# google-research/simclr

Measured on AMD Instinct MI355X. Metric: images/sec (whole node), ResNet-50 1x SimCLR pretraining step @224px, higher is better.
Workload: dtype f32; 1 GPU; ResNet-50 1x, 224x224, 2 views/image, per-GPU batch 512, global batch 512, NT-Xent T=0.1 + linear-eval head + LARS, global BN, dp1; global_batch=512, parallelism=dp1

## Files before the change

### simclr_amd/csrc/conv.hip

```cpp
#include "common.h"
#include <stdlib.h>
#include <string.h>
#include <mutex>
#include <type_traits>

namespace {

enum { MODE_FWD = 0, MODE_DGRAD = 1 };

struct ConvP {
  const void* x;
  const void* w;
  void* y;
  float* stats;
  int V, IH, IW, IC, OH, OW, N, KH, KW, stride, pad;
  int pixpitch;
  int M, K;
  int nslot, accumulate;
  int m_tiles, n_tiles;
  int cs, py, px, cls_h, cls_w;
  int ntaps;
  int taps[9];
  unsigned long long tap_w, dy_w, dx_w;
  const void* bn_x;
  const void* bn_mask;
  const float *bn_scale, *bn_shift, *bn_mean, *bn_rstd;
  int bn_mode;
  const void* x2;
  const float* bias;
  int ic2, pixpitch2;
  int win_j, win_bytes;
  int fapply;
  const void* zero;
  int diag;
  int split;
  const float* pivot;
  int rem_full, rem_tiles, rem_parts;
  float* part_ws;
  unsigned* part_flags;
  unsigned* part_err;
  int w_ps;
  int x_ps;
  unsigned x_bytes;
  int rs_dq[3], rs_drow[3], rs_dcol[3];
};

#ifdef SIMCLR_DIAG
#define DIAG(b) ((p.diag & (b)) != 0)
#else
#define DIAG(b) false
#endif

template <typename T> struct MMA;
template <> struct MMA<uint16_t> {
  __device__ static __forceinline__ f32x4 run(const u32x4& a, const u32x4& b, f32x4 c) {
    return __builtin_amdgcn_mfma_f32_16x16x32_bf16(__builtin_bit_cast(bf16x8, a),
                                                   __builtin_bit_cast(bf16x8, b), c, 0, 0, 0);
  }
};
template <> struct MMA<float> {
  __device__ static __forceinline__ f32x4 run(const u32x4& a, const u32x4& b, f32x4 c) {
#pragma unroll
    for (int j = 0; j < 4; ++j)
      c = __builtin_amdgcn_mfma_f32_16x16x4f32(__uint_as_float(a[j]), __uint_as_float(b[j]), c, 0, 0, 0);
    return c;
  }
};

__device__ __forceinline__ void split_terms2(const u32x4& c0, const u32x4& c1, u32x4& hi, u32x4& lo) {
#pragma unroll
  for (int j = 0; j < 4; ++j) {
    const float x0 = __uint_as_float(j < 2 ? c0[2 * j] : c1[2 * j - 4]), x1 = __uint_as_float(j < 2 ? c0[2 * j + 1] : c1[2 * j - 3]);
    const uint32_t h = pack_bf16x2(x0, x1);
    hi[j] = h;
    lo[j] = pack_bf16x2(x0 - __uint_as_float(h << 16), x1 - __uint_as_float(h & 0xffff0000u));
  }
}
__device__ __forceinline__ void split_terms3(const u32x4& c0, const u32x4& c1, u32x4& hi, u32x4& lo, u32x4& lo2) {
#pragma unroll
  for (int j = 0; j < 4; ++j) {
    const float x0 = __uint_as_float(j < 2 ? c0[2 * j] : c1[2 * j - 4]), x1 = __uint_as_float(j < 2 ? c0[2 * j + 1] : c1[2 * j - 3]);
    const uint32_t h = pack_bf16x2(x0, x1);
    const float r0 = x0 - __uint_as_float(h << 16), r1 = x1 - __uint_as_float(h & 0xffff0000u);
    const uint32_t l = pack_bf16x2(r0, r1);
    hi[j] = h;
    lo[j] = l;
    lo2[j] = pack_bf16x2(r0 - __uint_as_float(l << 16), r1 - __uint_as_float(l & 0xffff0000u));
  }
}
__device__ __forceinline__ f32x4 mma_bf16(const u32x4& a, const u32x4& b, f32x4 c) {
  return __builtin_amdgcn_mfma_f32_16x16x32_bf16(__builtin_bit_cast(bf16x8, a), __builtin_bit_cast(bf16x8, b), c, 0, 0, 0);
}
typedef __attribute__((ext_vector_type(8))) _Float16 f16x8;
#define F16_WSCALE_LOG2 8
__device__ __forceinline__ void split_terms2_f16(const u32x4& c0, const u32x4& c1, u32x4& hi, u32x4& lo) {
#pragma unroll
  for (int j = 0; j < 4; ++j) {
    const float x0 = __uint_as_float(j < 2 ? c0[2 * j] : c1[2 * j - 4]), x1 = __uint_as_float(j < 2 ? c0[2 * j + 1] : c1[2 * j - 3]);
    uint32_t h, l;
    split_pair<true>(x0, x1, h, l);
    hi[j] = h; lo[j] = l;
  }
}
__device__ __forceinline__ f32x4 mma_f16(const u32x4& a, const u32x4& b, f32x4 c) {
  return __builtin_amdgcn_mfma_f32_16x16x32_f16(__builtin_bit_cast(f16x8, a), __builtin_bit_cast(f16x8, b), c, 0, 0, 0);
}
template <int NA, int NB, bool TR, int terms, bool PSA = false, bool PSB2 = false, typename LA, typename LB>
__device__ __forceinline__ void mma_f32_chunks(f32x4* __restrict__ accp, LA lda, LB ldb) {
  static_assert(terms == 0 || terms == 3 || terms == 6 || terms == 13, "0 = exact fp32, 3 / 6 = split-bf16 terms, 13 = three split-fp16 terms");
  static_assert(!(PSA || PSB2) || terms == 3 || terms == 13, "pre-split operand: two planes (hi, lo) = the three-term products only");
#define acc_(i, j) accp[TR ? (j) * NA + (i) : (i) * NB + (j)]
  if constexpr (terms == 0) {
#pragma unroll
    for (int ks = 0; ks < 2; ++ks) {
      u32x4 a[NA], b[NB];
#pragma unroll
      for (int i = 0; i < NA; ++i) a[i] = lda(i, ks);
#pragma unroll
      for (int j = 0; j < NB; ++j) b[j] = ldb(j, ks);
#pragma unroll
      for (int i = 0; i < NA; ++i)
#pragma unroll
        for (int j = 0; j < NB; ++j)
#pragma unroll
          for (int e = 0; e < 4; ++e)
            acc_(i, j) = __builtin_amdgcn_mfma_f32_16x16x4f32(__uint_as_float(a[i][e]), __uint_as_float(b[j][e]), acc_(i, j), 0, 0, 0);
    }
// ... 1149 lines not shown
                const u32x2 mv = *(const u32x2*)((const uint16_t*)p.bn_mask + off + n);
                mk[0] = __uint_as_float(mv[0] << 16); mk[1] = __uint_as_float(mv[0] & 0xffff0000u);
                mk[2] = __uint_as_float(mv[1] << 16); mk[3] = __uint_as_float(mv[1] & 0xffff0000u);
              }
            } else {
              const float4 sc = *(const float4*)(bnp + nl), sh = *(const float4*)(bnp + BN + nl);
              mk[0] = fmaf(xf[0], sc.x, sh.x); mk[1] = fmaf(xf[1], sc.y, sh.y);
              mk[2] = fmaf(xf[2], sc.z, sh.z); mk[3] = fmaf(xf[3], sc.w, sh.w);
            }
            const float4 mu = *(const float4*)(bnp + 2 * BN + nl), rs = *(const float4*)(bnp + 3 * BN + nl);
            const float mua[4] = {mu.x, mu.y, mu.z, mu.w}, rsa[4] = {rs.x, rs.y, rs.z, rs.w};
#pragma unroll
            for (int r = 0; r < 4; ++r) {
              v[r] = mk[r] > 0.f ? v[r] : 0.f;
              st_s[ni][r] += v[r];
              st_q[ni][r] += v[r] * (xf[r] - mua[r]) * rsa[r];
            }
          }
          if (sizeof(T) == 4) {
            *(float4*)dst = make_float4(v[0], v[1], v[2], v[3]);
          } else {
            u32x2 pk; pk[0] = pack_bf16x2(v[0], v[1]); pk[1] = pack_bf16x2(v[2], v[3]);
            *(u32x2*)dst = pk;
          }
        }
      }
    }
    }
  }
  if (ROWSTATS) {
    __syncthreads();
    float* red = WSUM ? (float*)wred : (float*)smem;
    constexpr int NRED = WSUM ? NW : RPP;
    if (!WSUM) {
#pragma unroll
      for (int e = 0; e < 8; ++e) {
        red[((tid / CPR) * BN + e_cc * 8 + e) * 2] = e_s[e];
        red[((tid / CPR) * BN + e_cc * 8 + e) * 2 + 1] = e_q[e];
      }
      __syncthreads();
    }
    const bool own_slot = p.nslot >= mslots;
    if (tid < BN && n0 + tid < p.N && (count > 0 || own_slot)) {
      float s1 = 0.f, s2 = 0.f;
      for (int w = 0; w < NRED; ++w) { s1 += red[(w * BN + tid) * 2]; s2 += red[(w * BN + tid) * 2 + 1]; }
      if (BNEPI) s2 = (s2 - bnp[2 * BN + tid] * s1) * bnp[3 * BN + tid];
      float* st = p.stats + (long long)(own_slot ? mslot : mslot % p.nslot) * 2 * p.N;
      if (own_slot) { st[n0 + tid] = s1; st[p.N + n0 + tid] = s2; }
      else { atomicAdd(st + n0 + tid, s1); atomicAdd(st + p.N + n0 + tid, s2); }
    }
    return;
  }
  if (STATS) {
    __syncthreads();
    float* red = (float*)smem;
#pragma unroll
    for (int ni = 0; ni < NI; ++ni) {
#pragma unroll
      for (int r = 0; r < 4; ++r) {
        float s = st_s[ni][r], ss = st_q[ni][r];
#pragma unroll
        for (int o = 1; o < 16; o <<= 1) { s += __shfl_xor(s, o, 64); ss += __shfl_xor(ss, o, 64); }
        if (fl == 0) {
          const int nl = wn * 64 + ni * 16 + g * 4 + r;
          red[(wm * BN + nl) * 2] = s;
          red[(wm * BN + nl) * 2 + 1] = ss;
        }
      }
    }
    __syncthreads();
    const bool own_slot = p.nslot >= mslots;
    if (tid < BN && n0 + tid < p.N && (count > 0 || own_slot)) {
      float s = 0.f, ss = 0.f;
#pragma unroll
      for (int w = 0; w < WM; ++w) { s += red[(w * BN + tid) * 2]; ss += red[(w * BN + tid) * 2 + 1]; }
      float* st = p.stats + (long long)(own_slot ? mslot : mslot % p.nslot) * 2 * p.N;
      if (own_slot) { st[n0 + tid] = s; st[p.N + n0 + tid] = ss; }
      else { atomicAdd(st + n0 + tid, s); atomicAdd(st + p.N + n0 + tid, ss); }
    }
  }
}

#include "igemm_wide.h"

struct WgradP {
  const void* x;
  const void* dy;
  float* dw;
  int V, IH, IW, IC, OH, OW, N, KH, KW, stride, pad, pixpitch;
  int M, K, splits, chunks_per_split;
  int k_tiles, n_tiles;
  int xcd_map;
  const void* zero;
  int diag;
  int split;
  int dy_ps;
};

typedef __attribute__((ext_vector_type(4))) short s16x4_t;
typedef __attribute__((address_space(3))) s16x4_t lds_s16x4_t;

template <typename T> __device__ __forceinline__ int px_key(int px) {
  return sizeof(T) == 2 ? ((px & 3) | (((px >> 3) & 1) << 2)) : (((px & 3) << 1) | ((px >> 2) & 1));
}

template <typename T, int BKW, int BNW, bool MT = false>
__global__ __launch_bounds__(256) void conv_wgrad(const WgradP p) {
  constexpr int EPC = Elem<T>::EPC;
  constexpr int BR = 8 * EPC;
  constexpr int WK = 2;
  constexpr int WNN = 2;
  constexpr int KI = BKW / WK / 16;
  constexpr int NI = BNW / WNN / 16;
  constexpr int A_CPR = BKW / EPC;
  constexpr int B_CPR = BNW / EPC;
  constexpr int A_CH = BR * A_CPR / 256;
  constexpr int B_CH = BR * B_CPR / 256;
  constexpr int A_RB = BKW * sizeof(T);
  constexpr int B_RB = BNW * sizeof(T);
  constexpr int A_BLK = A_RB / 32;
  constexpr int B_BLK = B_RB / 32;
  constexpr int BUF = BR * (A_RB + B_RB);
  extern __shared__ __attribute__((aligned(16))) unsigned char smem[];

  const int tid = threadIdx.x, lane = tid & 63;
  const int wave = __builtin_amdgcn_readfirstlane(tid >> 6);
  const int g = lane >> 4, fl = lane & 15;
  const int wk = wave / WNN, wn = wave % WNN;
  const int tiles = p.k_tiles * p.n_tiles;
  int tile, split;
  if (p.xcd_map) {
    const int xcd = blockIdx.x & 7, bidx = blockIdx.x >> 3;
    tile = bidx % tiles;
    split = (bidx / tiles) * 8 + xcd;
  } else {
    tile = blockIdx.x % tiles;
    split = blockIdx.x / tiles;
  }
  if (split >= p.splits) return;
  const int ktile = tile % p.k_tiles;
  const int ntile = tile / p.k_tiles;
  const int kk0 = ktile * BKW;
  const int tap = kk0 / p.IC, ci0 = kk0 - tap * p.IC;
  const int ty = tap / p.KW, tx = tap - ty * p.KW;
  const int n0 = ntile * BNW;
  const T* __restrict__ X = (const T*)p.x;
  const T* __restrict__ DY = (const T*)p.dy;

  f32x4 acc[KI][NI];
#pragma unroll
  for (int i = 0; i < KI; ++i)
#pragma unroll
    for (int j = 0; j < NI; ++j) acc[i][j] = (f32x4){0.f, 0.f, 0.f, 0.f};

  const int nchunks = (p.M + BR - 1) / BR;
  const int c_begin = split * p.chunks_per_split;
  const int c_end = min(nchunks, c_begin + p.chunks_per_split);

  u32x4 ra[A_CH], rb[B_CH];
#ifdef SIMCLR_DIAG
#pragma unroll
  for (int j = 0; j < A_CH; ++j) ra[j] = zero16();
#pragma unroll
  for (int j = 0; j < B_CH; ++j) rb[j] = zero16();
#endif
  const bool flat = p.KH == 1 && p.KW == 1 && p.stride == 1 && p.pad == 0 && p.IH == p.OH && p.IW == p.OW;
// ... 1439 lines not shown
__global__ __launch_bounds__(256) void presplit_packed(const float4* __restrict__ src, u32x4* __restrict__ dst, long long npix) {
  for (long long i = blockIdx.x * 256ll + threadIdx.x; i < npix; i += (long long)gridDim.x * 256ll) {
    const float4 v = src[i];
    uint32_t h0, l0, h1, l1;
    split_pair<false>(v.x, v.y, h0, l0);
    split_pair<false>(v.z, v.w, h1, l1);
    dst[i] = (u32x4){h0, h1, l0, l1};
  }
}

__global__ void unpack_stem_dw(const float* __restrict__ src, float* __restrict__ dst, int KH, int KW,
                               int CI, int CO, int KWP, int accumulate) {
  const int total = KH * KW * CI * CO;
  for (int i = blockIdx.x * blockDim.x + threadIdx.x; i < total; i += gridDim.x * blockDim.x) {
    const int co = i % CO;
    const int ci = (i / CO) % CI;
    const int kw = (i / (CO * CI)) % KW;
    const int kh = i / (CO * CI * KW);
    const float v = src[(long long)((kh * KWP + kw) * 4 + ci) * CO + co];
    dst[i] = accumulate ? dst[i] + v : v;
  }
}

static int g_f32_terms_fwd = 0, g_f32_terms_bwd = 0;
static bool valid_terms(int t, bool fwd) { return t == 0 || t == 3 || t == 6 || (fwd && t == 13); }
static int terms_of(int* dtype, bool fwd) {
  const int f = (*dtype >> 12) & 0xff;
  *dtype &= ~(0xff << 12);
  if (f == 0) return fwd ? g_f32_terms_fwd : g_f32_terms_bwd;
  return valid_terms(f - 1, fwd) ? f - 1 : -1;
}

static bool take_ps_w(int* dtype) {
  const bool f = (*dtype & SIMCLR_FMT_PS_W) != 0;
  *dtype &= ~SIMCLR_FMT_PS_W;
  return f;
}

static thread_local char g_last_inst[512] = "";
static bool dry_run() { return simclr_dry_run(); }
template <typename T, int MODE> static void record_inst(const char* kern, unsigned grid, unsigned block, size_t lds, const ConvP& p) {
  snprintf(g_last_inst, sizeof(g_last_inst), "(%s) elt=%d role=%s grid=%u block=%u lds=%zu m_tiles=%d n_tiles=%d tail_parts=%d", kern,
           (int)sizeof(T), MODE == MODE_FWD ? "fwd" : "dgrad", grid, block, lds, p.m_tiles, p.n_tiles, p.rem_parts);
}
template <typename T> static const char* type_name() { return sizeof(T) == 2 ? "uint16_t" : "float"; }
static const char* mode_name(int mode) { return mode == MODE_FWD ? "MODE_FWD" : "MODE_DGRAD"; }
static const char* tf(bool v) { return v ? "true" : "false"; }

template <typename T, int MODE, int BN, bool STATS, bool GLDS>
static void run_igemm(dim3 grid, dim3 block, size_t lds, hipStream_t stream, const ConvP& p) {
  char name[128];
  snprintf(name, sizeof(name), "conv_igemm<%s, %s, %d, %s, %s>", type_name<T>(), mode_name(MODE), BN, tf(STATS), tf(GLDS));
  record_inst<T, MODE>(name, grid.x, block.x, lds, p);
  if (!dry_run()) hipLaunchKernelGGL((conv_igemm<T, MODE, BN, STATS, GLDS>), grid, block, lds, stream, p);
}

template <int MODE, bool STATS, bool BNEPI, bool FLAT>
static void run_wide(dim3 grid, dim3 block, size_t lds, hipStream_t stream, const ConvP& p) {
  char name[128];
  snprintf(name, sizeof(name), "conv_igemm_wide<%s, %s, %s, %s>", mode_name(MODE), tf(STATS), tf(BNEPI), tf(FLAT));
  record_inst<uint16_t, MODE>(name, grid.x, block.x, lds, p);
  if (!dry_run()) hipLaunchKernelGGL((conv_igemm_wide<MODE, STATS, BNEPI, FLAT>), grid, block, lds, stream, p);
}

template <typename T, int MODE, int BM, int BN, int NW, int STAGES, bool STATS, bool BNEPI, bool EXT = false,
          bool WIN = false, bool FAPPLY = false, int SPL = 0, bool TAIL = false, bool PSB = false, int FAS = 0, int EPS = 0, bool PSX = false>
static void run_persistent(dim3 grid, dim3 block, size_t lds, hipStream_t stream, const ConvP& p) {
  const int opt[9] = {EXT, WIN, FAPPLY, SPL, TAIL, PSB, FAS, EPS, PSX};
  const bool is_bool[9] = {true, true, true, false, true, true, false, false, true};
  int n = 9;
  while (n > 0 && opt[n - 1] == 0) --n;
  char name[256];
  int len = snprintf(name, sizeof(name), "conv_igemm_persistent<%s, %s, %d, %d, %d, %d, %s, %s", type_name<T>(), mode_name(MODE), BM, BN, NW,
                     STAGES, tf(STATS), tf(BNEPI));
  for (int i = 0; i < n; ++i)
    len += is_bool[i] ? snprintf(name + len, sizeof(name) - len, ", %s", tf(opt[i])) : snprintf(name + len, sizeof(name) - len, ", %d", opt[i]);
  snprintf(name + len, sizeof(name) - len, ">");
  record_inst<T, MODE>(name, grid.x, block.x, lds, p);
  if (!dry_run())
    hipLaunchKernelGGL((conv_igemm_persistent<T, MODE, BM, BN, NW, STAGES, STATS, BNEPI, EXT, WIN, FAPPLY, SPL, TAIL, PSB, FAS, EPS, PSX>),
                       grid, block, lds, stream, p);
}

struct WgradRec { int k_tiles, n_tiles, splits, chunks_per_split, xcd_map; };
static WgradRec rec_of(const WgradP& p) { return {p.k_tiles, p.n_tiles, p.splits, p.chunks_per_split, p.xcd_map}; }
static WgradRec rec_of(const Wgrad3P& p) { return {p.ci_tiles, p.co_tiles, p.splits, p.chunks_per_split, 1}; }
static WgradRec rec_of(const StemWgP& p) { return {1, 1, p.splits, p.chunks_per_split, 0}; }
static void record_wgrad(const char* kern, int elt, const char* role, unsigned grid, unsigned block, size_t lds, const WgradRec& r) {
  snprintf(g_last_inst, sizeof(g_last_inst), "(%s) elt=%d role=%s grid=%u block=%u lds=%zu k_tiles=%d n_tiles=%d splits=%d chunks_per_split=%d xcd_map=%d",
           kern, elt, role, grid, block, lds, r.k_tiles, r.n_tiles, r.splits, r.chunks_per_split, r.xcd_map);
}

template <typename T, int BKW, int BNW, bool MT = false>
static void run_wgrad(const char* role, unsigned grid, unsigned block, size_t lds, hipStream_t stream, const WgradP& p) {
  char name[128];
  snprintf(name, sizeof(name), MT ? "conv_wgrad<%s, %d, %d, true>" : "conv_wgrad<%s, %d, %d>", type_name<T>(), BKW, BNW);
  record_wgrad(name, (int)sizeof(T), role, grid, block, lds, rec_of(p));
  if (!dry_run()) hipLaunchKernelGGL((conv_wgrad<T, BKW, BNW, MT>), dim3(grid), dim3(block), lds, stream, p);
}

template <typename T, int BKW, int BNW, int BRM, int STAGES, int WK = 2, int WNN = 2, bool GRAM = false, bool MT = false, int SPL = 0, int PSD = 0>
static void run_wgrad_dma(const char* role, unsigned grid, unsigned block, size_t lds, hipStream_t stream, const WgradP& p) {
  const int opt[6] = {WK, WNN, GRAM, MT, SPL, PSD}, dflt[6] = {2, 2, 0, 0, 0, 0};
  const bool is_bool[6] = {false, false, true, true, false, false};
  int n = 6;
  while (n > 0 && opt[n - 1] == dflt[n - 1]) --n;
  char name[160];
  int len = snprintf(name, sizeof(name), "conv_wgrad_dma<%s, %d, %d, %d, %d", type_name<T>(), BKW, BNW, BRM, STAGES);
  for (int i = 0; i < n; ++i)
    len += is_bool[i] ? snprintf(name + len, sizeof(name) - len, ", %s", tf(opt[i])) : snprintf(name + len, sizeof(name) - len, ", %d", opt[i]);
  snprintf(name + len, sizeof(name) - len, ">");
  record_wgrad(name, (int)sizeof(T), role, grid, block, lds, rec_of(p));
  if (!dry_run())
    hipLaunchKernelGGL((conv_wgrad_dma<T, BKW, BNW, BRM, STAGES, WK, WNN, GRAM, MT, SPL, PSD>), dim3(grid), dim3(block), lds, stream, p);
}

template <int ST> static void run_wgrad3x3_bf16(unsigned grid, unsigned block, size_t lds, hipStream_t stream, const Wgrad3P& q) {
  char name[64];
  snprintf(name, sizeof(name), "conv_wgrad3x3_bf16<%d>", ST);
  record_wgrad(name, 2, "wgrad", grid, block, lds, rec_of(q));
  if (!dry_run()) hipLaunchKernelGGL(conv_wgrad3x3_bf16<ST>, dim3(grid), dim3(block), lds, stream, q);
}
static void run_wgrad3x3_f32ps(unsigned grid, unsigned block, size_t lds, hipStream_t stream, const Wgrad3P& q) {
  record_wgrad("conv_wgrad3x3_f32ps", 4, "wgrad", grid, block, lds, rec_of(q));
  if (!dry_run()) hipLaunchKernelGGL(conv_wgrad3x3_f32ps, dim3(grid), dim3(block), lds, stream, q);
}
template <int STAGES> static void run_stem_wgrad_ps(unsigned grid, unsigned block, size_t lds, hipStream_t stream, const StemWgP& p) {
  char name[64];
  snprintf(name, sizeof(name), "stem_wgrad_ps<7, 2, %d>", STAGES);
  record_wgrad(name, 4, "stem_wgrad_ps", grid, block, lds, rec_of(p));
  if (!dry_run()) hipLaunchKernelGGL((stem_wgrad_ps<7, 2, STAGES>), dim3(grid), dim3(block), lds, stream, p);
}
static void run_slab_reduce(const void* slabs, int splits, long long numel, float* out, int accumulate, hipStream_t stream) {
  const int grid = max(1, (int)ceil_div(numel / 4, 16));
  const size_t len = strlen(g_last_inst);
  snprintf(g_last_inst + len, sizeof(g_last_inst) - len, " reduce_grid=%d", grid);
  if (!dry_run()) hipLaunchKernelGGL(slab_reduce, dim3(grid), dim3(256), 0, stream, (const float*)slabs, splits, numel, out, accumulate);
}

static const void* zero_page() {
  static void* zp = nullptr;
  if (dry_run()) return (const void*)&g_last_inst;
  if (!zp && hipGetSymbolAddress(&zp, HIP_SYMBOL(g_zero16)) != hipSuccess) zp = nullptr;
  return zp;
}

static void igemm_persistent_grid(long long M, int N, int* bn, int* n_tiles, int* grid, bool narrow = false) {
  const int BN = (N <= 64 || narrow) ? 64 : 128;
  const int m_tiles = (int)((M + 127) / 128);
  const int nt = ceil_div(N, BN);
  const int unit = 8 * nt;
  const int resident = (BN == 64 ? 3 : 2) * 256;
  int pg = (resident / unit) * unit;
  if (pg < unit) pg = unit;
  const int need = ceil_div(m_tiles, 8) * unit;
  if (pg > need) pg = need;
  *bn = BN; *n_tiles = nt; *grid = pg;
}

static bool igemm_use_256(const ConvP& p, bool fwd) {
  if (p.N % 256 != 0 || p.ntaps <= 0 || p.N / 256 > 32) return false;
  const char* e = getenv("SIMCLR_IGEMM_TILE");
  const int mode = e ? atoi(e) : 0;
  if (mode == 256) return true;
  if (mode == 128) return false;
  if (p.KH != 1 || p.KW != 1 || p.M < 150000) return false;
// ... 79 lines not shown
    if (sc->flags) (void)hipFree(sc->flags);
    sc->ws = nullptr; sc->flags = nullptr; sc->floats = 0; sc->nflags = 0;
    const size_t want_f = slots * tile_floats, want_n = slots < 1024 ? 1024 : slots;
    if (hipMalloc((void**)&sc->ws, want_f * sizeof(float)) != hipSuccess ||
        hipMalloc((void**)&sc->flags, (want_n + 1) * sizeof(unsigned)) != hipSuccess ||
        hipMemsetAsync(sc->flags, 0, (want_n + 1) * sizeof(unsigned), stream) != hipSuccess ||
        (lost && hipMemcpyAsync(sc->flags + want_n, &lost, sizeof(unsigned), hipMemcpyHostToDevice, stream) != hipSuccess) ||
        (lost && hipStreamSynchronize(stream) != hipSuccess)) {
      (void)hipGetLastError();
      if (sc->ws) (void)hipFree(sc->ws);
      if (sc->flags) (void)hipFree(sc->flags);
      sc->ws = nullptr; sc->flags = nullptr;
      return false;
    }
    sc->floats = want_f; sc->nflags = want_n;
  }
  p.part_ws = sc->ws; p.part_flags = sc->flags; p.part_err = sc->flags + sc->nflags;
  return true;
}

static int split_tail_timeouts(unsigned* host_total) {
  SIMCLR_CHECK_ARG(host_total != nullptr, "conv2d_split_tail_timeouts: null argument");
  std::lock_guard<std::mutex> lock(g_scratch_mutex);
  unsigned total = 0;
  for (int i = 0; i < g_split_scratch_n; ++i) {
    if (!g_split_scratch[i].flags) continue;
    unsigned v = 0;
    if (hipMemcpy(&v, g_split_scratch[i].flags + g_split_scratch[i].nflags, sizeof(unsigned), hipMemcpyDeviceToHost) != hipSuccess) {
      simclr_set_error("conv2d_split_tail_timeouts: %s", hipGetErrorString(hipGetLastError()));
      return 2;
    }
    total += v;
    if (v != 0 && hipMemset(g_split_scratch[i].flags, 0, g_split_scratch[i].nflags * sizeof(unsigned)) != hipSuccess) {
      simclr_set_error("conv2d_split_tail_timeouts: %s", hipGetErrorString(hipGetLastError()));
      return 2;
    }
  }
  *host_total = total;
  return 0;
}

struct PresplitScratch { hipStream_t stream; void* buf; size_t bytes; };
static PresplitScratch g_presplit[8];
static int g_presplit_n = 0;
static thread_local int g_last_presplit = 0;
static bool presplit_enabled(long long rows, int K) {
  const char* e = getenv("SIMCLR_F32_PRESPLIT");
  return !(e && atoi(e) == 0) && K % 32 == 0 && rows > 0;
}
static const void* presplit_weights(const void* w, long long rows, int K, hipStream_t stream, bool f16) {
  if (dry_run()) return w;
  std::lock_guard<std::mutex> lock(g_scratch_mutex);
  PresplitScratch* sc = nullptr;
  for (int i = 0; i < g_presplit_n; ++i)
    if (g_presplit[i].stream == stream) sc = &g_presplit[i];
  if (!sc) {
    if (g_presplit_n == 8) return nullptr;
    sc = &g_presplit[g_presplit_n++];
    *sc = PresplitScratch{stream, nullptr, 0};
  }
  const size_t need = (size_t)rows * K * sizeof(float);
  if (sc->bytes < need) {
    if (sc->buf) (void)hipFree(sc->buf);
    sc->buf = nullptr; sc->bytes = 0;
    const size_t want = need < (16u << 20) ? (16u << 20) : need;
    if (hipMalloc(&sc->buf, want) != hipSuccess) { (void)hipGetLastError(); sc->buf = nullptr; return nullptr; }
    sc->bytes = want;
  }
  const long long nblocks = rows * (K / 32);
  if (f16) hipLaunchKernelGGL(presplit_rows<true>, dim3((unsigned)ceil_div(nblocks * 8, 256)), dim3(256), 0, stream,
                              (const float*)w, (uint32_t*)sc->buf, nblocks, (float)(1 << F16_WSCALE_LOG2));
  else hipLaunchKernelGGL(presplit_rows<false>, dim3((unsigned)ceil_div(nblocks * 8, 256)), dim3(256), 0, stream,
                          (const float*)w, (uint32_t*)sc->buf, nblocks, 1.0f);
  return sc->buf;
}

struct IgemmPlan {
  enum Family {
    EMPTY,
    UNSUPPORTED,
    WIDE,
    TILE256,
    TILE128,
    FALLBACK,
  } family = EMPTY;
  ConvP p;
  int bn = 0, spl = 0, fas = 0, eps = 0;
  bool stats = false, bnepi = false, ext = false, win = false, fapply = false, tail = false, psb = false, psx = false;
  bool flat = false;
  unsigned grid = 0, block = 0;
  size_t lds = 0;
  size_t tile_floats = 0;
  bool presplit = false;
};

template <typename T, int MODE>
static IgemmPlan plan_igemm(const ConvP& p0, bool can_split, bool can_presplit) {
  constexpr bool bf16 = sizeof(T) == 2, fwd = MODE == MODE_FWD;
  IgemmPlan k;
  ConvP& p = k.p;
  p = p0;
  const bool narrow = igemm_narrow(p, sizeof(T), !fwd);
  const int BN = (p.N <= 64 || narrow) ? 64 : 128;
  p.m_tiles = ceil_div(p.M, 128);
  p.n_tiles = ceil_div(p.N, BN);
  if (p.M <= 0) return k;
#ifdef SIMCLR_DIAG
  { const char* e = getenv("SIMCLR_DIAG"); p.diag = e ? atoi(e) : 0; }
#endif
  const bool st = p.stats != nullptr;
  k.bnepi = p.bn_mode != 0;
  k.ext = p.x2 != nullptr;
  k.stats = k.bnepi || (st && !k.ext);
  if (p.ntaps <= 0 || p.n_tiles > 64) {
    if (p.x_ps || (p.w_ps && p.ntaps > 0) || p.accumulate == 2) { k.family = IgemmPlan::UNSUPPORTED; return k; }
    k.family = IgemmPlan::FALLBACK;
    k.bn = BN; k.stats = st; k.bnepi = k.ext = false;
    k.grid = ceil_div(p.m_tiles, 8) * 8 * p.n_tiles; k.block = 256;
    k.lds = 2 * (128 + BN) * 128;
    const size_t epi = 128 * (BN * 2 + 8) + 128 * sizeof(long long);
    if (bf16 && epi > k.lds) k.lds = epi;
    return k;
  }
  const bool wide = bf16 && igemm_use_wide(p, fwd);
  if (wide || (bf16 && igemm_use_256(p, fwd))) {
    p.m_tiles = ceil_div(p.M, 256);
    p.n_tiles = p.N / 256;
    const int unit = 8 * p.n_tiles;
    k.grid = min(max(unit, (256 / unit) * unit), ceil_div(p.m_tiles, 8) * unit);
    k.block = 512;
    k.tile_floats = (size_t)256 * 256;
    if (wide) {
      k.family = IgemmPlan::WIDE;
      p.x_bytes = (unsigned)((long long)p.V * p.IH * p.IW * p.pixpitch * 2);
      const int dist[3] = {8, 128, 136}, chw = p.cls_h * p.cls_w;
      for (int i = 0; i < 3; ++i) {
        p.rs_dq[i] = dist[i] / chw;
        const int r = dist[i] - p.rs_dq[i] * chw;
        p.rs_drow[i] = r / p.cls_w; p.rs_dcol[i] = r - p.rs_drow[i] * p.cls_w;
      }
      k.lds = 131072 + 4 * 256 * sizeof(float) + 256 * sizeof(long long) + 8 * 256 * 2 * sizeof(float) + 4 * 512 * sizeof(int);
      if (can_split) split_tail_plan(p, k.grid, p.ntaps * (p.IC / 64), 1, true);
      k.flat = p.KH == 1 && p.KW == 1 && p.stride == 1 && p.pad == 0 && p.cs == 1 && p.IH == p.OH && p.IW == p.OW;
    } else {
      k.family = IgemmPlan::TILE256;
      k.bn = 256;
      k.lds = 2 * (256 + 256) * 128 + 5 * 256 * sizeof(float) + 256 * sizeof(long long) + 8 * 256 * 2 * sizeof(float);
      k.fapply = p.fapply != 0;
      if (k.fapply) k.stats = k.bnepi = k.ext = false;
      else if (can_split) split_tail_plan(p, k.grid, p.ntaps * (p.IC / 64) + (p.x2 ? p.ic2 / 64 : 0), 1);
      k.tail = p.rem_parts >= 2;
    }
    return k;
  }
  k.family = IgemmPlan::TILE128;
  k.bn = BN;
  int pg, bn_, nt_;
  igemm_persistent_grid(p.M, p.N, &bn_, &nt_, &pg, narrow);
  k.grid = pg; k.block = 256;
  k.lds = 2 * (128 + BN) * 128 + 5 * BN * sizeof(float) + 128 * sizeof(long long);
  const bool win3 = (bf16 || p.split == 3 || p.split == 13) && !p.fapply && !p.x2 && p.KH == 3 && p.KW == 3 && p.stride == 1 &&
                    p.pad == 1 && p.cs == 1 && p.ntaps == 9 && p.IH == p.OH && p.IW == p.OW && p.IW <= 62 && p.accumulate < 2;
  const int bk_elems = 128 / (int)sizeof(T);
  if (bf16 && BN == 128 && !p.fapply && can_split) {
    split_tail_plan(p, pg, win3 ? p.IC / bk_elems : p.ntaps * (p.IC / bk_elems) + (p.x2 ? p.ic2 / bk_elems : 0), win3 ? 9 : 1);
    k.tile_floats = (size_t)128 * BN;
  } else {
    p.rem_parts = 0;
  }
  k.tail = p.rem_parts >= 2;
  if (!bf16) {
    const bool presplit = can_presplit && presplit_enabled(p.N, p.K);
    if (!fwd && p.split == 3) { k.psb = true; k.presplit = !p.w_ps && presplit; }
    if (fwd && p.split == 13) { k.psb = true; k.presplit = !p.w_ps && presplit; }
    if (k.psb && !p.w_ps && !presplit) {
      k.psb = false;
      if (fwd) p.split = 6;
    }
    if ((p.x_ps && !k.psb) || (p.w_ps && !k.psb)) { k.family = IgemmPlan::UNSUPPORTED; return k; }
    k.spl = k.psb || p.split == 3 || p.split == 6 ? p.split : 0;
    k.psx = k.psb && p.x_ps;
  }
  if (p.fapply) {
    k.fapply = true;
    k.stats = k.bnepi = k.ext = false;
    if (bf16 && p.bn_x && p.bn_mode && p.bn_mask && (p.N & 31) == 0) k.fas = p.bn_mean ? 2 : 1;
    return k;
  }
  int eps = 0;
  if (bf16 && !fwd && p.bn_mode && !k.tail) {
    if (p.bn_mode == 2 && !p.accumulate) eps = 1;
    else if (p.bn_mode == 4) eps = p.accumulate ? 4 : 3;
  }
  k.win = bf16 ? win3 : win3 && k.psb && (fwd ? !p.bn_mode : p.x_ps && (p.bn_mode != 0) == st);
  if (!bf16 && !fwd && k.psb && k.spl == 3 && k.psx && !k.ext && (p.bn_mode == 2 || p.bn_mode == 4) && p.accumulate < 2 && (p.N & 63) == 0 &&
      ((uintptr_t)p.bn_mask & 15) == 0 && f32_eps_exists(k.win, 1 + (p.bn_mode == 4 ? 2 : 0) + p.accumulate) && f32_epi_batch())
    eps = 1 + (p.bn_mode == 4 ? 2 : 0) + p.accumulate;
  if (k.win) {
    const int rows = ((128 + 2 * (p.IW + 1)) + 31) / 32 * 32;
    p.win_j = rows / 32;
    p.win_bytes = (!bf16 || rows * 128 > 128 * BN * 2) ? rows * 128 : 128 * BN * 2;
    k.lds = (size_t)p.win_bytes + 2 * BN * 128 + 5 * BN * sizeof(float) + 128 * sizeof(long long) + 128;
    k.eps = (!bf16 || eps == 1) ? eps : 0;
  } else {
    k.eps = !bf16 || eps == 1 || (!k.ext && eps >= 3) ? eps : 0;
    if (k.psx && k.ext) k.family = IgemmPlan::UNSUPPORTED;
  }
  return k;
}

template <typename V, V... Vs> struct among {};
template <typename F> static bool with_consts(F&& f) { return f(); }
template <typename V, V... Vs, typename... Rest, typename F>
static bool with_consts(F&& f, among<V, Vs...>, V x, Rest... rest) {
  bool hit = false;
  (void)((x == Vs && (hit = with_consts([&](auto... c) { return f(std::integral_constant<V, Vs>{}, c...); }, rest...), true)) || ...);
  return hit;
}
using Bools = among<bool, false, true>;

static constexpr bool epilogue_exists(bool st, bool be, bool ex) { return (st || !be) && (!ex || st == be); }
static constexpr bool tile128_exists(bool bf16, bool fwd, int bn, bool st, bool be, bool ex, bool win, bool fa, int spl, bool tail,
                                     bool psb, int fas, int eps, bool psx) {
  if (fa)
    return fwd && !st && !be && !ex && !win && !tail && !eps && !psx && (bf16 ? spl == 0 && !psb : fas == 0 && psb == (spl == 13));
  if (fas || !epilogue_exists(st, be, ex) || (win && ex)) return false;
  if (bf16)
    return spl == 0 && !psb && !psx && (eps ? st && be && !tail && (eps == 1 || (!ex && !win && (eps == 3 || eps == 4))) : !tail || bn == 128);
  if (tail) return false;
  if (eps) return !fwd && st && be && psb && spl == 3 && !ex && psx && f32_eps_exists(win, eps);
  if (win) return psb && (fwd ? spl == 13 && !be && !psx : spl == 3 && psx);
  if (psx) return !fwd && !ex && psb && spl == 3;
  if (psb) return fwd ? spl == 13 && !be && !ex : spl == 3;
  return spl == 0 || spl == 3 || spl == 6;
}

template <typename T, int MODE>
static bool launch_plan(const IgemmPlan& k, hipStream_t s) {
  constexpr bool bf16 = sizeof(T) == 2, fwd = MODE == MODE_FWD;
  const dim3 g(k.grid), b(k.block);
  switch (k.family) {
    case IgemmPlan::FALLBACK:
      return with_consts([&](auto BN, auto ST) { run_igemm<T, MODE, BN, ST, true>(g, b, k.lds, s, k.p); return true; },
                         among<int, 64, 128>{}, k.bn, Bools{}, k.stats);
    case IgemmPlan::WIDE:
      if constexpr (bf16)
        return with_consts([&](auto ST, auto BE, auto FLAT) {
          if constexpr (!epilogue_exists(ST, BE, false)) return false;
          else { run_wide<MODE, ST, BE, FLAT>(g, b, k.lds, s, k.p); return true; }
        }, Bools{}, k.stats, Bools{}, k.bnepi, Bools{}, k.flat);
      return false;
    case IgemmPlan::TILE256:
      if constexpr (bf16)
        return with_consts([&](auto ST, auto BE, auto EX, auto FA, auto TAIL) {
          if constexpr (FA ? !(fwd && !ST && !BE && !EX && !TAIL) : !epilogue_exists(ST, BE, EX)) return false;
          else { run_persistent<T, MODE, 256, 256, 8, 2, ST, BE, EX, false, FA, 0, TAIL>(g, b, k.lds, s, k.p); return true; }
        }, Bools{}, k.stats, Bools{}, k.bnepi, Bools{}, k.ext, Bools{}, k.fapply, Bools{}, k.tail);
      return false;
    case IgemmPlan::TILE128: {
      using Spl = std::conditional_t<bf16, among<int, 0>, among<int, 0, 3, 6, 13>>;
      using FpBools = std::conditional_t<bf16, among<bool, false>, Bools>;
      using HBools = std::conditional_t<bf16, Bools, among<bool, false>>;
      using Fas = std::conditional_t<bf16, among<int, 0, 1, 2>, among<int, 0>>;
      using Eps = std::conditional_t<bf16, among<int, 0, 1, 3, 4>, among<int, 0>>;
      if constexpr (!bf16 && !fwd) {
        if (k.eps)
          return k.stats && k.bnepi && !k.ext && !k.win && !k.fapply && k.spl == 3 && !k.tail && k.psb && !k.fas && k.psx &&
                 with_consts([&](auto BN, auto EPS) {
                   static_assert(f32_eps_exists(false, EPS), "the list below = the epilogues f32_eps_exists names");
                   run_persistent<T, MODE, 128, BN, 4, 2, true, true, false, false, false, 3, false, true, 0, EPS, true>(g, b, k.lds, s, k.p);
                   return true;
                 }, among<int, 64, 128>{}, k.bn, among<int, 1, 4>{}, k.eps);
      }
      return with_consts([&](auto BN, auto ST, auto BE, auto EX, auto WIN, auto FA, auto SPL, auto TAIL, auto PSB, auto FAS, auto EPS, auto PSX) {
        if constexpr (!tile128_exists(bf16, fwd, BN, ST, BE, EX, WIN, FA, SPL, TAIL, PSB, FAS, EPS, PSX)) return false;
        else { run_persistent<T, MODE, 128, BN, 4, 2, ST, BE, EX, WIN, FA, SPL, TAIL, PSB, FAS, EPS, PSX>(g, b, k.lds, s, k.p); return true; }
      }, among<int, 64, 128>{}, k.bn, Bools{}, k.stats, Bools{}, k.bnepi, Bools{}, k.ext, Bools{}, k.win, Bools{}, k.fapply, Spl{}, k.spl,
         HBools{}, k.tail, FpBools{}, k.psb, Fas{}, k.fas, Eps{}, k.eps, FpBools{}, k.psx);
    }
    default:
      return false;
  }
}

template <typename T, int MODE>
static int launch_igemm_one(const ConvP& p, hipStream_t stream) {
  bool can_split = true, can_presplit = true;
  IgemmPlan k = plan_igemm<T, MODE>(p, can_split, can_presplit);
  if (k.family == IgemmPlan::UNSUPPORTED) return 1;
  if (k.p.rem_parts >= 2 && !split_tail_scratch(k.p, k.tile_floats, stream)) k = plan_igemm<T, MODE>(p, can_split = false, can_presplit);
  if (k.presplit) {
    const void* ws = presplit_weights(k.p.w, k.p.N, k.p.K, stream, k.spl == 13);
    if (ws) k.p.w = ws;
    else k = plan_igemm<T, MODE>(p, can_split, can_presplit = false);
  }
  if (k.family == IgemmPlan::EMPTY) return 0;
  if (k.family == IgemmPlan::UNSUPPORTED) return 1;
  if (k.family != IgemmPlan::FALLBACK) g_last_split_parts = k.p.rem_parts;
  if (sizeof(T) == 4 && MODE == MODE_DGRAD && k.family == IgemmPlan::TILE128) g_last_presplit = k.psb;
  return launch_plan<T, MODE>(k, stream) ? 0 : 1;
}

template <typename T, int MODE>
static int launch_igemm(const ConvP& p0, hipStream_t stream) {
  ConvP p = p0;
  if (MODE == MODE_FWD || p.stride == 1) {
    p.cs = 1; p.py = 0; p.px = 0; p.cls_h = p.OH; p.cls_w = p.OW;
    p.ntaps = p.KH * p.KW;
    p.tap_w = p.dy_w = p.dx_w = 0;
    for (int t = 0; t < p.ntaps; ++t) {
      p.taps[t] = t;
      const int ty = t / p.KW, tx = t % p.KW;
      const int dy = (MODE == MODE_FWD) ? ty : p.pad - ty, dx = (MODE == MODE_FWD) ? tx : p.pad - tx;
      p.tap_w |= (unsigned long long)t << (4 * t);
      p.dy_w |= (unsigned long long)(dy + 8) << (4 * t);
      p.dx_w |= (unsigned long long)(dx + 8) << (4 * t);
    }
    p.M = p.V * p.OH * p.OW;
    return launch_igemm_one<T, MODE>(p, stream);
  }
  const int S = p.stride;
  ConvP cls[4];
  int n = 0;
  for (int py = 0; py < S; ++py)
    for (int px = 0; px < S; ++px) {
      ConvP q = p;
      q.cs = S; q.py = py; q.px = px;
      q.cls_h = (p.OH - py + S - 1) / S;
      q.cls_w = (p.OW - px + S - 1) / S;
      q.ntaps = 0;
      q.tap_w = q.dy_w = q.dx_w = 0;
      for (int ty = 0; ty < p.KH; ++ty)
        for (int tx = 0; tx < p.KW; ++tx)
          if ((py + p.pad - ty) % S == 0 && (px + p.pad - tx) % S == 0 && q.ntaps < 9) {
            q.tap_w |= (unsigned long long)(ty * p.KW + tx) << (4 * q.ntaps);
            q.dy_w |= (unsigned long long)((py + p.pad - ty) / S + 8) << (4 * q.ntaps);
            q.dx_w |= (unsigned long long)((px + p.pad - tx) / S + 8) << (4 * q.ntaps);
            q.taps[q.ntaps++] = ty * p.KW + tx;
          }
      q.M = p.V * q.cls_h * q.cls_w;
      if (q.ntaps == 0 && p.accumulate == 2 && ((py | px) & 1)) q.accumulate = 0;
      else if (q.ntaps == 0 && p.accumulate) continue;
      if (p.accumulate == 3) q.accumulate = 0;
      if (q.ntaps == 0) q.x_ps = 0;
      if (plan_igemm<T, MODE>(q, true, true).family == IgemmPlan::UNSUPPORTED) return 1;
      cls[n++] = q;
    }
  for (int i = 0; i < n; ++i)
    if (int rc = launch_igemm_one<T, MODE>(cls[i], stream)) return rc;
  return 0;
}

struct ConvCall { int dtype, terms; bool w_ps, x_ps; };
static int conv_call(const char* fn, int dtype, bool fwd, int ps_w_terms, bool ps_in, int Cout, ConvCall* c) {
  c->terms = terms_of(&dtype, fwd);
  SIMCLR_CHECK_ARG(c->terms >= 0, "%s: bad matrix-arithmetic field in dtype (SIMCLR_FMT_TERMS)", fn);
  c->w_ps = ps_w_terms && take_ps_w(&dtype);
  SIMCLR_CHECK_ARG(!c->w_ps || ((dtype & 0xff) == SIMCLR_DT_F32 && c->terms == ps_w_terms),
                   "%s: pre-split weights (SIMCLR_FMT_PS_W) need fp32 storage and terms %d", fn, ps_w_terms);
  c->x_ps = ps_in && (dtype & SIMCLR_FMT_PS_IN) != 0;
  if (ps_in) dtype &= 0xff;
  SIMCLR_CHECK_ARG(!c->x_ps || (dtype == SIMCLR_DT_F32 && c->terms == 3 && Cout % 32 == 0),
// ... 685 lines not shown
```

Measured before the change: 3820 images/s.

## Add n-walk fp32 1x1 conv kernel that reuses input panel across output-channel tiles

Adds a specialized forward kernel for flat 1x1 fp32 convolutions with small input channels (64/128) and a fused BN-apply/residual/ReLU/mask tail. It stages a 64-row input panel in LDS once, splits it into f16 hi/lo terms, and walks all output-channel tiles of a group over it while streaming double-buffered weight tiles. The goal is to avoid re-reading and re-splitting the activation panel for every N tile, at the cost of more LDS and a new planning path. It is enabled by default through an env toggle.

```diff
diff --git a/simclr_amd/csrc/conv.hip b/simclr_amd/csrc/conv.hip
--- a/simclr_amd/csrc/conv.hip
+++ b/simclr_amd/csrc/conv.hip
@@ -43,6 +43,7 @@
   int x_ps;
   unsigned x_bytes;
   int rs_dq[3], rs_drow[3], rs_dcol[3];
+  int nw_groups, nw_gw;
 };
 
 #ifdef SIMCLR_DIAG
@@ -1358,6 +1359,7 @@
 }
 
 #include "igemm_wide.h"
+#include "igemm_nwalk.h"
 
 struct WgradP {
   const void* x;
@@ -2963,6 +2965,16 @@
                        grid, block, lds, stream, p);
 }
 
+template <int KPT, int FAS>
+static void run_nwalk(dim3 grid, dim3 block, size_t lds, hipStream_t stream, const ConvP& p) {
+  char name[64];
+  snprintf(name, sizeof(name), "conv_igemm_nwalk<%d, %d>", KPT, FAS);
+  record_inst<float, MODE_FWD>(name, grid.x, block.x, lds, p);
+  const size_t len = strlen(g_last_inst);
+  snprintf(g_last_inst + len, sizeof(g_last_inst) - len, " walk=n_inner n_group=%d n_groups=%d", p.nw_gw, p.nw_groups);
+  if (!dry_run()) hipLaunchKernelGGL((conv_igemm_nwalk<KPT, FAS>), grid, block, lds, stream, p);
+}
+
 struct WgradRec { int k_tiles, n_tiles, splits, chunks_per_split, xcd_map; };
 static WgradRec rec_of(const WgradP& p) { return {p.k_tiles, p.n_tiles, p.splits, p.chunks_per_split, p.xcd_map}; }
 static WgradRec rec_of(const Wgrad3P& p) { return {p.ci_tiles, p.co_tiles, p.splits, p.chunks_per_split, 1}; }
@@ -3208,6 +3220,7 @@
     WIDE,
     TILE256,
     TILE128,
+    NWALK,
     FALLBACK,
   } family = EMPTY;
   ConvP p;
@@ -3219,6 +3232,35 @@
   size_t tile_floats = 0;
   bool presplit = false;
 };
+
+static bool igemm_nwalk_on() {
+  const char* e = getenv("SIMCLR_IGEMM_NWALK");
+  return !e || atoi(e) != 0;
+}
+
+static void plan_nwalk(IgemmPlan& k) {
+  ConvP& p = k.p;
+  const bool flat = p.KH == 1 && p.KW == 1 && p.stride == 1 && p.pad == 0 && p.cs == 1 && p.IH == p.OH && p.IW == p.OW;
+  if (!igemm_nwalk_on() || !flat || !k.fapply || !k.psb || k.spl != 13 || k.psx || p.x2 || (p.IC != 64 && p.IC != 128) || p.K != p.IC ||
+      p.pixpitch < p.IC || (p.pixpitch & 3) || (p.N & 63) || p.N <= 128 || p.N > 512 || !p.bn_x || !p.bn_mode || !p.bn_mask ||
+      ((uintptr_t)p.bn_mask & 15) || p.rem_parts >= 2)
+    return;
+  const int m_tiles = ceil_div(p.M, 64);
+  int groups = 1;
+  while (m_tiles * groups < 2 * 3 * 256 && (p.N / groups) % 128 == 0) groups *= 2;
+  const int gw = p.N / groups;
+  const size_t lds = (size_t)(p.IC / 32) * 64 * 128 + 2 * 64 * 128 + (p.bn_mean ? 4 : 2) * gw * sizeof(float);
+  const int per_cu = 3 * lds <= 160 * 1024 ? 3 : 2;
+  const int unit = 8 * groups;
+  int pg = max(unit, (per_cu * 256 / unit) * unit);
+  const int need = ceil_div(m_tiles, 8) * unit;
+  if (pg > need) pg = need;
+  k.family = IgemmPlan::NWALK;
+  k.bn = 64; k.fas = p.bn_mean ? 2 : 1;
+  k.grid = pg; k.block = 256; k.lds = lds;
+  p.m_tiles = m_tiles; p.n_tiles = p.N / 64;
+  p.nw_groups = groups; p.nw_gw = gw;
+}
 
 template <typename T, int MODE>
 static IgemmPlan plan_igemm(const ConvP& p0, bool can_split, bool can_presplit) {
@@ -3311,6 +3353,7 @@
     k.fapply = true;
     k.stats = k.bnepi = k.ext = false;
     if (bf16 && p.bn_x && p.bn_mode && p.bn_mask && (p.N & 31) == 0) k.fas = p.bn_mean ? 2 : 1;
+    if (!bf16 && fwd) plan_nwalk(k);
     return k;
   }
   int eps = 0;
@@ -3404,6 +3447,11 @@
       }, among<int, 64, 128>{}, k.bn, Bools{}, k.stats, Bools{}, k.bnepi, Bools{}, k.ext, Bools{}, k.win, Bools{}, k.fapply, Spl{}, k.spl,
          HBools{}, k.tail, FpBools{}, k.psb, Fas{}, k.fas, Eps{}, k.eps, FpBools{}, k.psx);
     }
+    case IgemmPlan::NWALK:
+      if constexpr (!bf16 && fwd)
+        return with_consts([&](auto KPT, auto FAS) { run_nwalk<KPT, FAS>(g, b, k.lds, s, k.p); return true; },
+                           among<int, 2, 4>{}, k.p.IC / 32, among<int, 1, 2>{}, k.fas);
+      return false;
     default:
       return false;
   }
diff --git a/simclr_amd/csrc/igemm_nwalk.h b/simclr_amd/csrc/igemm_nwalk.h
--- /dev/null
+++ b/simclr_amd/csrc/igemm_nwalk.h
@@ -0,0 +1,128 @@
+template <int KPT, int FAS>
+__global__ __launch_bounds__(256, 3) void conv_igemm_nwalk(const ConvP p) {
+  static_assert((KPT == 2 || KPT == 4) && (FAS == 1 || FAS == 2), "IC = 64 | 128; fused-tail option sets 1 | 2");
+  constexpr int BM = 64, BN = 64, NI = BN / 16;
+  constexpr int PJ = KPT * BM / 32;
+  constexpr int NBP = FAS == 2 ? 4 : 2;
+  extern __shared__ __attribute__((aligned(16))) unsigned char smem[];
+  u32x4* Pn = (u32x4*)smem;
+  u32x4* Rg = Pn + KPT * BM * 8;
+  float* bnp = (float*)(Rg + 2 * BN * 8);
+  typedef __attribute__((address_space(1))) const void* gptr_t;
+  typedef __attribute__((address_space(3))) void* lptr_t;
+
+  const int tid = threadIdx.x, lane = tid & 63;
+  const int wave = __builtin_amdgcn_readfirstlane(tid >> 6);
+  const int g = lane >> 4, fl = lane & 15;
+  const float* __restrict__ X = (const float*)p.x;
+  const float* __restrict__ Wt = (const float*)p.w;
+  float* __restrict__ Y = (float*)p.y;
+  const int G = p.nw_gw, ngt = G / BN;
+  const int xcd = blockIdx.x & 7, l = blockIdx.x >> 3;
+  const int grp = l % p.nw_groups;
+  const int mslots = gridDim.x / p.nw_groups;
+  const int mslot = (l / p.nw_groups) * 8 + xcd;
+  const int ng0 = grp * G;
+  const int count = (mslot < p.m_tiles) ? (p.m_tiles - mslot + mslots - 1) / mslots : 0;
+  const int kc = (lane & 7) ^ (lane >> 3);
+
+  for (int i = tid; i < G; i += 256) {
+    const int n = ng0 + i;
+    bnp[i] = p.bn_scale[n];
+    bnp[G + i] = p.bn_shift[n];
+    if (FAS == 2) { bnp[2 * G + i] = p.bn_mean[n]; bnp[3 * G + i] = p.bn_rstd[n]; }
+  }
+
+  auto issue_panel = [&](int mt) __attribute__((always_inline)) {
+#pragma unroll
+    for (int j = 0; j < PJ; ++j) {
+      const int q = wave * PJ + j;
+      const int kt = q / (BM / 8), rg = q % (BM / 8);
+      const int m = mt * BM + 8 * rg + (lane >> 3);
+      const void* src = m < p.M ? (const void*)(X + (long long)m * p.pixpitch + kt * 32 + kc * 4) : p.zero;
+      __builtin_amdgcn_global_load_lds((gptr_t)src, (lptr_t)(smem + q * 1024), 16, 0, 0);
+    }
+  };
+  auto issue_w = [&](int nt, int kt, int b) __attribute__((always_inline)) {
+    unsigned char* dst = (unsigned char*)(Rg + b * BN * 8) + wave * 2048;
+#pragma unroll
+    for (int j = 0; j < 2; ++j) {
+      const int n = ng0 + nt * BN + 8 * (wave * 2 + j) + (lane >> 3);
+      __builtin_amdgcn_global_load_lds((gptr_t)(Wt + (long long)n * p.K + kt * 32 + kc * 4), (lptr_t)(dst + j * 1024), 16, 0, 0);
+    }
+  };
+  int wnt = 0, wkt = 0, issued = 0, buf = 0;
+  const int total = count * ngt * KPT;
+  auto issue_next_w = [&]() __attribute__((always_inline)) {
+    issue_w(wnt, wkt, issued & 1);
+    ++issued;
+    if (++wkt == KPT) { wkt = 0; if (++wnt == ngt) wnt = 0; }
+  };
+  if (count > 0) {
+    issue_panel(mslot);
+    issue_next_w();
+  }
+  for (int ct = 0; ct < count; ++ct) {
+    const int m = (mslot + ct * mslots) * BM + wave * 16 + fl;
+    const long long off = m < p.M ? (long long)m * p.N : -1;
+    for (int nt = 0; nt < ngt; ++nt) {
+      f32x4 acc[NI];
+#pragma unroll
+      for (int ni = 0; ni < NI; ++ni) acc[ni] = (f32x4){0.f, 0.f, 0.f, 0.f};
+#pragma unroll
+      for (int kt = 0; kt < KPT; ++kt) {
+        asm volatile("s_waitcnt vmcnt(0)" ::: "memory");
+        __syncthreads();
+        if (issued < total) issue_next_w();
+        if (nt == 0 && kt == 0) {
+          for (int q = tid; q < KPT * BM * 4; q += 256) {
+            const int row = q >> 2, gq = q & 3;
+            u32x4* w0 = Pn + row * 8 + (gq ^ (row & 7));
+            u32x4* w1 = Pn + row * 8 + ((4 + gq) ^ (row & 7));
+            u32x4 hi, lo;
+            split_terms2_f16(*w0, *w1, hi, lo);
+            *w0 = hi; *w1 = lo;
+          }
+          __syncthreads();
+        }
+        const u32x4* Bt = Rg + buf * BN * 8;
+        const u32x4* Pk = Pn + kt * BM * 8;
+        mma_f32_chunks<NI, 1, false, 13, true, true>(&acc[0],
+            [&](int i, int ks) { const int r = i * 16 + fl; return Bt[r * 8 + ((ks * 4 + g) ^ (r & 7))]; },
+            [&](int, int ks) { const int r = wave * 16 + fl; return Pk[r * 8 + ((ks * 4 + g) ^ (r & 7))]; });
+        buf ^= 1;
+      }
+      if (nt == ngt - 1 && ct + 1 < count) {
+        __syncthreads();
+        issue_panel(mslot + (ct + 1) * mslots);
+      }
+#pragma unroll
+      for (int ni = 0; ni < NI; ++ni) acc[ni] *= (1.0f / (float)(1 << F16_WSCALE_LOG2));
+      const bool ok = off >= 0;
+      const int nl0 = nt * BN + g * 4;
+      const long long a = ok ? off + ng0 + nl0 : 0;
+      float4 rr[NI];
+#pragma unroll
+      for (int ni = 0; ni < NI; ++ni) rr[ni] = *(const float4*)((const float*)p.bn_x + a + ni * 16);
+      u32x4 mbits;
+#pragma unroll
+      for (int ni = 0; ni < NI; ++ni) {
+        const int nl = nl0 + ni * 16;
+        const float4 sc = *(const float4*)(bnp + nl), sh = *(const float4*)(bnp + G + nl);
+        float o[4] = {fmaf(acc[ni][0], sc.x, sh.x), fmaf(acc[ni][1], sc.y, sh.y), fmaf(acc[ni][2], sc.z, sh.z), fmaf(acc[ni][3], sc.w, sh.w)};
+        const float4 r = rr[ni];
+        if (FAS == 2) {
+          const float4 rs = *(const float4*)(bnp + 2 * G + nl), rb = *(const float4*)(bnp + 3 * G + nl);
+          o[0] += fmaf(r.x, rs.x, rb.x); o[1] += fmaf(r.y, rs.y, rb.y); o[2] += fmaf(r.z, rs.z, rb.z); o[3] += fmaf(r.w, rs.w, rb.w);
+        } else { o[0] += r.x; o[1] += r.y; o[2] += r.z; o[3] += r.w; }
+#pragma unroll
+        for (int e = 0; e < 4; ++e) o[e] = fmaxf(o[e], 0.f);
+        if (ok) *(float4*)(Y + a + ni * 16) = make_float4(o[0], o[1], o[2], o[3]);
+        const unsigned bits = (o[0] > 0.f ? 1u : 0u) | (o[1] > 0.f ? 2u : 0u) | (o[2] > 0.f ? 4u : 0u) | (o[3] > 0.f ? 8u : 0u);
+        const unsigned b1 = __shfl(bits, lane + 16, 64), b2 = __shfl(bits, lane + 32, 64), b3 = __shfl(bits, lane + 48, 64);
+        mbits[ni] = bits | (b1 << 8) | (b2 << 16) | (b3 << 24);
+      }
+      if (ok && g == 0) *(u32x4*)((unsigned char*)p.bn_mask + (a >> 2)) = mbits;
+    }
+  }
+}
```

New measurement: 3873 images/s (median of 6 runs). 1.4% higher.
